# Xharlie/BtcDet

Measured on AMD Instinct MI355X. Metric: scenes/s fwd+bwd KITTI-Car bs=2/GPU (BtcDet hot path), higher is better.
Workload: dtype f32

## Files before the change

btcdet_amd/csrc/bn.hip:

```cpp
#include "btc_common.h"
#include "bn_fuse.h"
#include "../../include/btcdet_hip_infer.h"

#include <type_traits>

namespace {

constexpr int BN_T = 256;

struct BnShape {
  int N, C, cpow, rpi;
};

__device__ __forceinline__ void st_partial(double* p, double v) { btc_st_agent(p, v); }

template <bool BF, int W>
__device__ __forceinline__ void bn_ld(const float* base, long long i, float (&e)[W]) {
  if constexpr (W == 4) {
    const float4 v = btc_ld4<BF>(base, i);
    e[0] = v.x; e[1] = v.y; e[2] = v.z; e[3] = v.w;
  } else {
    e[0] = btc_ld1<BF>(base, i);
  }
}
// ... 14 lines not shown
#pragma unroll
      for (int q = 0; q < Q; ++q) s[q][tid * W + j] = acc[q][j];
    __syncthreads();
    if (rr == 0 && cw < S.C) {
      for (int l = 1; l < S.rpi; ++l)
#pragma unroll
        for (int j = 0; j < W; ++j)
#pragma unroll
          for (int q = 0; q < Q; ++q) acc[q][j] += s[q][(tid + l * S.cpow) * W + j];
      emit(cw, acc);
    }
    __syncthreads();
  }
}

template <int W, int Q, int D, class Rows, class Done>
__device__ __forceinline__ bool bn_reduce(const BnShape& S, const BnShape& SW, double* __restrict__ partial, int32_t* __restrict__ counter,
                                          Rows rows, Done done) {
  __shared__ double s[Q][BN_T * W];
  const int G = (int)gridDim.x;
  auto at = [&](int g, int q, int c) { return &partial[((size_t)g * Q + q) * S.C + c]; };
  bn_pass<W>(SW, s,
             [&](int cw, int rr, double (&acc)[Q][W]) { rows(cw, (long long)blockIdx.x * SW.rpi + rr, (long long)G * SW.rpi, acc); },
             [&](int cw, double (&acc)[Q][W]) {
#pragma unroll
               for (int j = 0; j < W; ++j)
#pragma unroll
                 for (int q = 0; q < Q; ++q) st_partial(at(blockIdx.x, q, cw * W + j), acc[q][j]);
             });
  if (!btc_last_arriver(counter, G)) return false;
  bn_pass<1>(S, s,
             [&](int c, int rr, double (&acc)[Q][1]) {
               int g = rr;
               for (; g + (D - 1) * S.rpi < G; g += D * S.rpi) {
                 double v[Q][D];
#pragma unroll
                 for (int u = 0; u < D; ++u)
#pragma unroll
                   for (int q = 0; q < Q; ++q) v[q][u] = btc_ld_agent(at(g + u * S.rpi, q, c));
#pragma unroll
                 for (int q = 0; q < Q; ++q) {
#pragma unroll
                   for (int h = 1; h < D; h *= 2)
#pragma unroll
                     for (int u = 0; u < D; u += 2 * h) v[q][u] += v[q][u + h];
                   acc[q][0] += v[q][0];
                 }
               }
               for (; g < G; g += S.rpi)
#pragma unroll
                 for (int q = 0; q < Q; ++q) acc[q][0] += btc_ld_agent(at(g, q, c));
             },
             [&](int c, double (&acc)[Q][1]) {
               double t[Q];
#pragma unroll
               for (int q = 0; q < Q; ++q) t[q] = acc[q][0];
               done(c, t);
             });
  if (threadIdx.x == 0) __hip_atomic_store(counter, 0, __ATOMIC_RELAXED, __HIP_MEMORY_SCOPE_AGENT);
  return true;
}

template <bool BF, bool VEC>
__global__ __launch_bounds__(BN_T) void bn_stats(const float* __restrict__ x, BnShape S, BnShape SW, double* __restrict__ partial,
                                                 int32_t* __restrict__ counter, float momentum, float eps, float* __restrict__ running_mean,
                                                 float* __restrict__ running_var, long long* __restrict__ num_batches,
                                                 float* __restrict__ mean_out, float* __restrict__ rstd_out) {
  constexpr int W = VEC ? 4 : 1;
  const bool last = bn_reduce<W, 2, 8>(
      S, SW, partial, counter,
      [&](int cw, long long r, long long stride, double (&acc)[2][W]) {
        const long long step = stride * S.C;
        long long i = r * S.C + cw * W;
// ... 55 lines not shown
      float g = gamma ? gamma[c + j] : 1.f, b = beta ? beta[c + j] : 0.f;
      o[j] = bn_affine(o[j], mean[c + j], rstd[c + j], g, b, relu);
    }
    btc_st4<BF>(y, i, o[0], o[1], o[2], o[3]);
  } else {
    int c = (int)(i % C);
    float g = gamma ? gamma[c] : 1.f, b = beta ? beta[c] : 0.f;
    btc_st1<BF>(y, i, bn_affine(btc_ld1<BF>(x, i), mean[c], rstd[c], g, b, relu));
  }
}

template <bool BF, bool VEC>
__global__ __launch_bounds__(BN_T) void bn_bwd_stats(const float* __restrict__ x, const float* __restrict__ y, const float* __restrict__ dy,
                                                     const float* __restrict__ mean, const float* __restrict__ rstd, BnShape S, BnShape SW, int relu,
                                                     double* __restrict__ partial, int32_t* __restrict__ counter,
                                                     float* __restrict__ dgamma, float* __restrict__ dbeta) {
  constexpr int W = VEC ? 4 : 1, U = VEC ? 2 : 4;
  bn_reduce<W, 2, 8>(
      S, SW, partial, counter,
      [&](int cw, long long r, long long stride, double (&acc)[2][W]) {
        float m[W], rs[W];
#pragma unroll
        for (int j = 0; j < W; ++j) { m[j] = mean[cw * W + j]; rs[j] = rstd[cw * W + j]; }
        const long long step = stride * S.C;
        long long i = r * S.C + cw * W;
        for (; r + (U - 1) * stride < S.N; r += U * stride, i += U * step) {
          float gv[U][W], yv[U][W], xv[U][W];
#pragma unroll
          for (int u = 0; u < U; ++u) {
            bn_ld<BF>(dy, i + u * step, gv[u]);
            bn_ld<BF>(y, i + u * step, yv[u]);
// ... 12 lines not shown
          float gv[W], yv[W], xv[W];
          bn_ld<BF>(dy, i, gv);
          bn_ld<BF>(y, i, yv);
          bn_ld<BF>(x, i, xv);
#pragma unroll
          for (int j = 0; j < W; ++j) {
            const float g = (relu && !(yv[j] > 0.f)) ? 0.f : gv[j];
            acc[0][j] += (double)g;
            acc[1][j] += (double)g * ((xv[j] - m[j]) * rs[j]);
          }
        }
      },
      [&](int c, const double (&t)[2]) {
        dbeta[c] = (float)t[0];
        dgamma[c] = (float)t[1];
      });
}

template <bool VEC, bool BF>
__global__ __launch_bounds__(BN_T) void bn_bwd_apply(const float* __restrict__ x, const float* __restrict__ y, const float* __restrict__ dy,
                                                     const float* __restrict__ mean, const float* __restrict__ rstd,
                                                     const float* __restrict__ gamma, const float* __restrict__ dgamma,
                                                     const float* __restrict__ dbeta, long long total, int C, int N, int relu, int training,
                                                     float* __restrict__ dx) {
  long long i = ((long long)blockIdx.x * blockDim.x + threadIdx.x) * (VEC ? 4 : 1);
  if (i >= total) return;
  const float invn = 1.0f / (float)N;
  constexpr int W = VEC ? 4 : 1;
  float xv[W], yv[W], gv[W];
  if (VEC) {
    float4 a = btc_ld4<BF>(x, i), b = btc_ld4<BF>(y, i), c4 = btc_ld4<BF>(dy, i);
    xv[0] = a.x; xv[W > 1 ? 1 : 0] = a.y; xv[W > 2 ? 2 : 0] = a.z; xv[W > 3 ? 3 : 0] = a.w;
    yv[0] = b.x; yv[W > 1 ? 1 : 0] = b.y; yv[W > 2 ? 2 : 0] = b.z; yv[W > 3 ? 3 : 0] = b.w;
    gv[0] = c4.x; gv[W > 1 ? 1 : 0] = c4.y; gv[W > 2 ? 2 : 0] = c4.z; gv[W > 3 ? 3 : 0] = c4.w;
  } else {
    xv[0] = btc_ld1<BF>(x, i); yv[0] = btc_ld1<BF>(y, i); gv[0] = btc_ld1<BF>(dy, i);
  }
  const int c = (int)(i % C);
  float o[W];
#pragma unroll
  for (int j = 0; j < W; ++j) {
    float g = gv[j];
    if (relu && !(yv[j] > 0.f)) g = 0.f;
    const float gm = gamma ? gamma[c + j] : 1.f, rs = rstd[c + j];
    if (training) {
      float xh = (xv[j] - mean[c + j]) * rs;
      o[j] = gm * rs * (g - dbeta[c + j] * invn - xh * dgamma[c + j] * invn);
    } else {
      o[j] = gm * rs * g;
    }
  }
  if (VEC) btc_st4<BF>(dx, i, o[0], o[W > 1 ? 1 : 0], o[W > 2 ? 2 : 0], o[W > 3 ? 3 : 0]);
  else btc_st1<BF>(dx, i, o[0]);
}

template <bool BF>
__global__ __launch_bounds__(BN_T) void col_sum(const float* __restrict__ x, BnShape S, double* __restrict__ partial,
                                                int32_t* __restrict__ counter, float* __restrict__ out) {
  bn_reduce<1, 1, 1>(
      S, S, partial, counter,
      [&](int c, long long r, long long stride, double (&acc)[1][1]) {
        for (; r + 3 * stride < S.N; r += 4 * stride) {
          float v0 = btc_ld1<BF>(x, r * S.C + c), v1 = btc_ld1<BF>(x, (r + stride) * S.C + c), v2 = btc_ld1<BF>(x, (r + 2 * stride) * S.C + c),
                v3 = btc_ld1<BF>(x, (r + 3 * stride) * S.C + c);
          acc[0][0] += ((double)v0 + (double)v1) + ((double)v2 + (double)v3);
        }
        for (; r < S.N; r += stride) acc[0][0] += (double)btc_ld1<BF>(x, r * S.C + c);
      },
// ... 39 lines not shown
};

template <class F>
int bn_by_width(int N, int C, F&& f) {
  if ((C & 3) == 0) return f(std::integral_constant<int, 4>(), bn_shape(N, C >> 2));
  return f(std::integral_constant<int, 1>(), bn_shape(N, C));
}

}

extern "C" size_t btc_bn_ws_bytes(int C) { return 256 + btc_align((size_t)512 * 2 * C * sizeof(double)); }

template <bool BF>
static int bn_fwd_impl(const float* x, int N, int C, const float* gamma, const float* beta, float* running_mean,
                               float* running_var, long long* num_batches_tracked, float momentum, float eps, int training, int relu,
                               float* y, float* save_mean, float* save_rstd, void* ws_, size_t ws_bytes, void* stream_, bool have_stats = false) {
  hipStream_t stream = (hipStream_t)stream_;
  BTC_CHECK_ARG(N >= 1 && C >= 1, "btc_bn_relu_fwd: empty input");
  BTC_CHECK_ARG(ws_bytes >= btc_bn_ws_bytes(C), "btc_bn_relu_fwd: workspace too small");
  BTC_CHECK_ARG(training || (running_mean && running_var), "btc_bn_relu_fwd: eval mode needs running statistics");
  const BnWs ws(ws_);
  const BnShape S = bn_shape(N, C);
  const long long total = (long long)N * C;
  return bn_by_width(N, C, [&](auto w, const BnShape& SW) {
    constexpr int W = decltype(w)::value;
    if (!have_stats && training) {
      const int g = W == 4 ? bn_grid_bytes(total * (BF ? 2 : 4), BTC_TUNE_BN_FWD_KB, 64) : bn_grid(N, S);
      bn_stats<BF, W == 4><<<g, BN_T, 0, stream>>>(x, S, SW, ws.partial, ws.counter, momentum, eps, running_mean, running_var,
                                                    num_batches_tracked, save_mean, save_rstd);
    } else if (!have_stats) {
      bn_eval_stats<<<btc_cdiv(C, BN_T), BN_T, 0, stream>>>(running_mean, running_var, C, eps, save_mean, save_rstd);
    }
    BTC_LAUNCH_CHECK();
    bn_apply<W == 4, BF><<<btc_cdiv(total / W, BN_T), BN_T, 0, stream>>>(x, save_mean, save_rstd, gamma, beta, total, C, relu, y);
    BTC_LAUNCH_CHECK();
    return BTC_OK;
  });
}

template <bool BF>
static int bn_bwd_impl(const float* x, const float* y, const float* dy, int N, int C, const float* gamma, const float* save_mean,
                               const float* save_rstd, int training, int relu, float* dx, float* dgamma, float* dbeta, void* ws_,
                               size_t ws_bytes, void* stream_) {
  hipStream_t stream = (hipStream_t)stream_;
  BTC_CHECK_ARG(N >= 1 && C >= 1, "btc_bn_relu_bwd: empty input");
  BTC_CHECK_ARG(ws_bytes >= btc_bn_ws_bytes(C), "btc_bn_relu_bwd: workspace too small");
  const BnWs ws(ws_);
  const BnShape S = bn_shape(N, C);
  const long long total = (long long)N * C;
  return bn_by_width(N, C, [&](auto w, const BnShape& SW) {
    constexpr int W = decltype(w)::value;
    const int g = W == 4 ? bn_grid_bytes(total * (BF ? 6 : 12), BTC_TUNE_BN_BWD_KB, 128) : bn_grid_bwd(N, S);
    bn_bwd_stats<BF, W == 4><<<g, BN_T, 0, stream>>>(x, y, dy, save_mean, save_rstd, S, SW, relu, ws.partial, ws.counter, dgamma, dbeta);
    BTC_LAUNCH_CHECK();
    bn_bwd_apply<W == 4, BF><<<btc_cdiv(total / W, BN_T), BN_T, 0, stream>>>(x, y, dy, save_mean, save_rstd, gamma, dgamma, dbeta, total, C, N,
                                                                             relu, training, dx);
    BTC_LAUNCH_CHECK();
    return BTC_OK;
  });
}

template <bool BF>
static int col_sum_impl(const float* x, int N, int C, float* out, void* ws_, size_t ws_bytes, void* stream_) {
  hipStream_t stream = (hipStream_t)stream_;
  BTC_CHECK_ARG(N >= 1 && C >= 1, "btc_col_sum: empty input");
  BTC_CHECK_ARG(ws_bytes >= btc_bn_ws_bytes(C), "btc_col_sum: workspace too small");
  const BnWs ws(ws_);
  const BnShape S = bn_shape(N, C);
  col_sum<BF><<<bn_grid_bwd(N, S), BN_T, 0, stream>>>(x, S, ws.partial, ws.counter, out);
// ... 48 lines not shown

extern "C" int btc_conv_bn_relu_fwd_src(int operands, const void* src, long long src_rows, const void* W, const float* bias, const int32_t* nbr,
                                        const int32_t* order, int n_rows, int K, int Cin, int Cout, void* x, const float* gamma, const float* beta,
                                        float* running_mean, float* running_var, long long* num_batches_tracked, float momentum, float eps, int relu,
                                        void* y, float* save_mean, float* save_rstd, void* ws, size_t ws_bytes, void* fuse_ws, void* stream) {
  BTC_CHECK_ARG(n_rows >= 1, "btc_conv_bn_relu_fwd: empty input");
  BTC_CHECK_ARG(operands >= BTC_OPERANDS_F32 && operands <= BTC_OPERANDS_F32_SPLIT, "btc_conv_bn_relu_fwd: operands=%d", operands);
  const bool bf = operands == BTC_OPERANDS_BF16_ACT || operands == BTC_OPERANDS_BF16;
  const bool fused = fuse_ws && Cout <= BN_FUSE_CMAX && btc_tune_get(BTC_TUNE_BN_FUSE) != 1;
  BnFuse bn = btc_bn_fuse_none();
  if (fused) {
    bn.counter = (int32_t*)fuse_ws;
    bn.slots = (double*)((char*)fuse_ws + 256);
    bn.mean_out = save_mean; bn.rstd_out = save_rstd;
    bn.running_mean = running_mean; bn.running_var = running_var; bn.num_batches = num_batches_tracked;
    bn.momentum = momentum; bn.eps = eps; bn.N = n_rows; bn.C = Cout; bn.nslots = btc_bn_fuse_nslots(n_rows);
  }
  const int rc = btc_apply("btc_conv_bn_relu_fwd_src", BTC_PASS_FWD, operands, src, src_rows, W, bias, nbr, order, n_rows, K, Cin, Cout, x,
                           (hipStream_t)stream, fused ? &bn : nullptr);
  if (rc) return rc;
  if (bf)
    return bn_fwd_impl<true>((const float*)x, n_rows, Cout, gamma, beta, running_mean, running_var, num_batches_tracked, momentum, eps, 1, relu,
                             (float*)y, save_mean, save_rstd, ws, ws_bytes, stream, fused);
  return bn_fwd_impl<false>((const float*)x, n_rows, Cout, gamma, beta, running_mean, running_var, num_batches_tracked, momentum, eps, 1, relu,
                            (float*)y, save_mean, save_rstd, ws, ws_bytes, stream, fused);
}

extern "C" int btc_conv_bn_eval_fwd(int operands, const void* src, long long src_rows, const void* W, const float* bias, const int32_t* nbr,
                                    const int32_t* order, int n_rows, int K, int Cin, int Cout, const float* gamma, const float* beta,
                                    const float* running_mean, const float* running_var, float eps, int relu, void* y, void* stream) {
  BTC_CHECK_ARG(n_rows >= 1, "btc_conv_bn_eval_fwd: empty input");
  BTC_CHECK_ARG(operands >= BTC_OPERANDS_F32 && operands <= BTC_OPERANDS_F32_SPLIT, "btc_conv_bn_eval_fwd: operands=%d", operands);
  BTC_CHECK_ARG(running_mean && running_var, "btc_conv_bn_eval_fwd: eval mode needs running statistics");
  BTC_CHECK_ARG(src && W && nbr && y, "btc_conv_bn_eval_fwd: null operand");
  BnFuse bn = btc_bn_fuse_none();
  bn.ev_mean = running_mean; bn.ev_var = running_var; bn.ev_gamma = gamma; bn.ev_beta = beta; bn.ev_relu = relu ? 1 : 0;
  bn.eps = eps; bn.N = n_rows; bn.C = Cout;
  return btc_apply("btc_conv_bn_eval_fwd", BTC_PASS_FWD, operands, src, src_rows, W, bias, nbr, order, n_rows, K, Cin, Cout, y, (hipStream_t)stream, &bn);
}
```

btcdet_amd/csrc/bn_fuse.h:

```cpp
#pragma once
#include "btc_common.h"

constexpr int BN_FUSE_SLOTS_MAX = 512;
constexpr int BN_FUSE_CMAX = 1024;

struct BnFuse {
  double* slots;
  int32_t* counter;
  float* mean_out;
  float* rstd_out;
  float* running_mean;
  float* running_var;
  long long* num_batches;
  float momentum, eps;
  int N, C;
  int nslots;
  const float* ev_mean;
  const float* ev_var;
  const float* ev_gamma;
  const float* ev_beta;
  int ev_relu;
};

static inline size_t btc_bn_fuse_bytes() { return 256 + (size_t)BN_FUSE_SLOTS_MAX * 2 * BN_FUSE_CMAX * sizeof(double); }

static inline int btc_bn_fuse_nslots(long long n_rows) {
  int s = 32;
  while (s < BN_FUSE_SLOTS_MAX && (long long)s * 1024 < n_rows) s <<= 1;
  return s;
}

static inline BnFuse btc_bn_fuse_none() {
  BnFuse b;
  b.slots = nullptr; b.counter = nullptr; b.mean_out = b.rstd_out = b.running_mean = b.running_var = nullptr; b.num_batches = nullptr;
  b.momentum = b.eps = 0.f; b.N = b.C = 0; b.nslots = 32;
  b.ev_mean = b.ev_var = b.ev_gamma = b.ev_beta = nullptr; b.ev_relu = 0;
  return b;
}

__device__ __forceinline__ float bn_rstd_eval(float running_var, float eps) { return 1.0f / sqrtf(__fadd_rn(running_var, eps)); }

__device__ __forceinline__ float bn_affine(float v, float mean, float rstd, float g, float b, int relu) {
  const float t = __fadd_rn(__fmul_rn(__fmul_rn(__fsub_rn(v, mean), rstd), g), b);
  return relu ? fmaxf(t, 0.f) : t;
}

struct BnEvalCol { float m, rs, g, b; };
__device__ __forceinline__ BnEvalCol bn_eval_col(const BnFuse& bn, int col) {
  BnEvalCol k;
  const bool in = col < bn.C;
// ... 17 lines not shown
      s2 += x * x;
    }
    s1 += __shfl_xor(s1, 16, 64);
    s2 += __shfl_xor(s2, 16, 64);
    s1 += __shfl_xor(s1, 32, 64);
    s2 += __shfl_xor(s2, 32, 64);
    const int col = col0 + nt * 16 + lane;
    if (lane < 16 && col < bn.C) {
      double* p = bn.slots + ((size_t)slot * 2) * BN_FUSE_CMAX + col;
      unsafeAtomicAdd(p, s1);
      unsafeAtomicAdd(p + BN_FUSE_CMAX, s2);
    }
  }
}

__device__ __forceinline__ void bn_fuse_finish(const BnFuse& bn, int* s_flag, double* s_part = nullptr) {
  const int tid = threadIdx.x;
  asm volatile("s_waitcnt vmcnt(0)" ::: "memory");
  __syncthreads();
  if (tid == 0) {
    const int total = (int)(gridDim.x * gridDim.y * gridDim.z);
    *s_flag = (btc_ticket_take(bn.counter) == total - 1);
  }
  __syncthreads();
  if (!*s_flag) return;
  if (tid == 0) btc_ticket_acquire();
  __syncthreads();
  auto publish = [&](int c, double a, double b) {
    const double mean = a / bn.N;
    double var = b / bn.N - mean * mean;
    if (var < 0.0) var = 0.0;
    bn.mean_out[c] = (float)mean;
    bn.rstd_out[c] = (float)(1.0 / sqrt(var + (double)bn.eps));
    if (bn.running_mean) {
      const double unb = bn.N > 1 ? var * ((double)bn.N / (double)(bn.N - 1)) : var;
      bn.running_mean[c] = (float)((1.0 - bn.momentum) * bn.running_mean[c] + bn.momentum * mean);
      bn.running_var[c] = (float)((1.0 - bn.momentum) * bn.running_var[c] + bn.momentum * unb);
    }
  };
  const int T = (int)blockDim.x;
  if (s_part && bn.C <= T) {
    const int G = T / bn.C;
    const int c = tid % bn.C, g = tid / bn.C;
    double a = 0.0, b = 0.0;
    if (g < G)
      for (int s = g; s < bn.nslots; s += G) {
        double* p = bn.slots + ((size_t)s * 2) * BN_FUSE_CMAX + c;
        a += btc_ld_agent(p);
        b += btc_ld_agent(p + BN_FUSE_CMAX);
        p[0] = 0.0;
        p[BN_FUSE_CMAX] = 0.0;
      }
    s_part[2 * tid] = a;
    s_part[2 * tid + 1] = b;
// ... 29 lines not shown
```

btcdet_amd/csrc/btc_common.h:

```cpp
#pragma once
#include <hip/hip_runtime.h>
#include <stdint.h>
#include <stdio.h>

#include "../../include/btcdet_hip.h"

#define BTC_EMPTY_KEY (-1)
#define BTC_EMPTY_IDX 0x7F7F7F7F

void btc_set_error(const char* fmt, ...);

#define BTC_CHECK_ARG(cond, ...)            \
  do {                                      \
    if (!(cond)) {                          \
      btc_set_error(__VA_ARGS__);           \
      return BTC_EINVAL;                    \
    }                                       \
  } while (0)

#define BTC_HIP(call)                                                             \
  do {                                                                            \
    hipError_t e_ = (call);                                                       \
    if (e_ != hipSuccess) {                                                       \
      btc_set_error("%s failed: %s (%s:%d)", #call, hipGetErrorString(e_), __FILE__, __LINE__); \
// ... 25 lines not shown
__device__ __forceinline__ void btc_ticket_acquire() { __builtin_amdgcn_fence(__ATOMIC_ACQUIRE, "agent"); }
__device__ __forceinline__ bool btc_last_arriver(int32_t* counter, int total) {
  __shared__ int s_last;
  asm volatile("s_waitcnt vmcnt(0)" ::: "memory");
  __syncthreads();
  if (threadIdx.x == 0) s_last = (btc_ticket_take(counter) == total - 1);
  __syncthreads();
  if (!s_last) return false;
  if (threadIdx.x == 0) btc_ticket_acquire();
  __syncthreads();
  return true;
}
#endif

#define BTC_TUNE_KEYS 24
int btc_tune_get(int key);

bool btc_apply_glds_supported(int K, int Cred, int Cres);
bool btc_apply_glds_has_shape(int shape, bool bf = false);
size_t btc_apply_glds_lds_bytes(int shape, int kc, int K, bool bf, int stages = 3);
int btc_apply_glds_stages(int shape, int kc, int K, bool bf, int asked);
int btc_launch_apply_glds(bool trans_w, int shape, int kc, int xcd, bool bf, const void* feat, const float* W, const float* bias,
                          const int32_t* nbr, const int32_t* order , int n_rows, int K, int Cred, int Cres, void* out,
                          hipStream_t stream, const struct BnFuse* bn = nullptr );

int btc_apply(const char* who, int pass, int operands, const void* src, long long src_rows, const void* W, const float* bias, const int32_t* nbr,
              const int32_t* order, int n_rows, int K, int Cin, int Cout, void* dst, hipStream_t stream, const struct BnFuse* bn);

int btc_apply_bf16w(const void* src, const void* Wq, const float* bias, const int32_t* nbr, const int32_t* order, int n_rows, int K, int Cred,
                    int Cres, void* dst, hipStream_t stream, int mirror = 0, const struct BnFuse* bn = nullptr);
// ... 112 lines not shown
```

btcdet_amd/csrc/conv_apply_bf16.hip:

```cpp
#include "conv_tile.h"

namespace {

__device__ unsigned short g_zero_row_b[128];

constexpr int B_STAGES = 3;

template <int WR, int WC, int NTW, int KC, bool PAIR = false>
__global__ __launch_bounds__(64 * WR * WC) void conv_apply_b(const unsigned short* __restrict__ feat, const unsigned short* __restrict__ Wq,
                                                             const float* __restrict__ bias, const int32_t* __restrict__ nbr,
                                                             const int32_t* __restrict__ order, int n_rows, int K, int Cred, int Cres,
                                                             unsigned short* __restrict__ out, int flags, const BnFuse bn) {
  extern __shared__ __attribute__((aligned(16))) char smem[];
  constexpr int NW = WR * WC, THREADS = 64 * NW;
  constexpr int TM = 16 * WR, TN = 16 * NTW * WC;
  constexpr int UPR = KC / 8;
  constexpr int RPB = (128 / (KC * 2)) < 1 ? 1 : (128 / (KC * 2));
  constexpr int A_UNITS = TM * UPR, B_UNITS = TN * UPR;
  constexpr int NAI_TOTAL = (A_UNITS + 63) / 64, NAI = (NAI_TOTAL + NW - 1) / NW;
  constexpr int NBI_TOTAL = (B_UNITS + 63) / 64, NBI = (NBI_TOTAL + NW - 1) / NW;
  constexpr int NPI = NAI + NBI;
  constexpr int A_BYTES = (TM * KC * 2 + 1023) / 1024 * 1024;
  constexpr int B_BYTES = (TN * KC * 2 + 1023) / 1024 * 1024;
  constexpr int STAGE = A_BYTES + B_BYTES;
// ... 85 lines not shown
        for (int nt = 0; nt < NTW; ++nt)
          acc[nt] = __builtin_amdgcn_mfma_f32_16x16x32_bf16(a[s], b[s][nt], acc[nt], 0, 0, 0);
      }
    }
    st = (st == B_STAGES - 1) ? 0 : st + 1;
  }

  float vals[NTW][4];
  bool valid[4];
  int rows[4];
#pragma unroll
  for (int r = 0; r < 4; ++r) rows[r] = s_row[wr * 16 + kq * 4 + r];
  apply_tile_epilogue<NTW>(acc, rows, n0 + wc * NTW * 16, bias, Cres, out, bn, bn.ev_mean != nullptr, vals, valid);
  if (bn.slots) {
    bn_fuse_wave<NTW>(bn, vals, valid, n0 + wc * NTW * 16, (int)((bx * WR + wr) & (bn.nslots - 1)));
    bn_fuse_finish(bn, (int*)smem, (double*)(smem + 16));
  }
}

size_t lds_bytes_b(int tm, int tn, int kc, int K) {
  const size_t a = ((size_t)tm * kc * 2 + 1023) / 1024 * 1024, b = ((size_t)tn * kc * 2 + 1023) / 1024 * 1024;
  return (size_t)B_STAGES * (a + b) + apply_tail_bytes(tm, K);
}

template <int WR, int WC, int NTW, int KC, bool PAIR = false>
int launch_b(const unsigned short* feat, const unsigned short* Wq, const float* bias, const int32_t* nbr, const int32_t* order, int n_rows, int K, int Cred,
             int Cres, unsigned short* out, int flags, hipStream_t stream, const BnFuse& bn) {
  constexpr int TM = 16 * WR, TN = 16 * NTW * WC;
  return apply_launch<conv_apply_b<WR, WC, NTW, KC, PAIR>>("conv_apply_b", dim3(btc_cdiv(n_rows, TM), Cres / TN), 64 * WR * WC, lds_bytes_b(TM, TN, KC, K),
                                                          stream, feat, Wq, bias, nbr, order, n_rows, K, Cred, Cres, out, flags, bn);
}
// ... 89 lines not shown
```

btcdet_amd/csrc/conv_apply_glds.hip:

```cpp
#include "conv_tile.h"

namespace {

__device__ float g_zero_row[64];

constexpr int G_STAGES_DEFAULT = 3;
constexpr int G_STAGES_MAX = 8;

__device__ __forceinline__ void transpose4(const f32x4 v, float& y0, float& y1, float& y2, float& y3) {
  unsigned x0 = __float_as_uint(v[0]), x1 = __float_as_uint(v[1]), x2 = __float_as_uint(v[2]), x3 = __float_as_uint(v[3]);
  auto a = __builtin_amdgcn_permlane32_swap(x0, x2, false, false);
  x0 = a[0]; x2 = a[1];
  auto b = __builtin_amdgcn_permlane32_swap(x1, x3, false, false);
  x1 = b[0]; x3 = b[1];
  auto c = __builtin_amdgcn_permlane16_swap(x0, x1, false, false);
  x0 = c[0]; x1 = c[1];
  auto d = __builtin_amdgcn_permlane16_swap(x2, x3, false, false);
  x2 = d[0]; x3 = d[1];
  y0 = __uint_as_float(x0); y1 = __uint_as_float(x1); y2 = __uint_as_float(x2); y3 = __uint_as_float(x3);
}

template <int WR, int WC, int NTW, bool TRANS_W, int KC, bool BF>
__global__ __launch_bounds__(64 * WR * WC) void conv_apply_g(const void* __restrict__ feat_, const float* __restrict__ W,
                                                             const float* __restrict__ bias, const int32_t* __restrict__ nbr,
// ... 162 lines not shown
      }
    }
    st = (st == S - 1) ? 0 : st + 1;
  }

  float vals[NTW][4];
  bool valid[4];
  int rows[4];
#pragma unroll
  for (int r = 0; r < 4; ++r) rows[r] = s_row[wr * 16 + kq * 4 + r];
  const bool ev = !TRANS_W && bn.ev_mean != nullptr;
  typedef typename std::conditional<BF, unsigned short, float>::type OUT;
  apply_tile_epilogue<NTW>(acc, rows, n0 + wc * NTW * 16, bias, Cres, (OUT*)out_, bn, ev, vals, valid);
  if (bn.slots) {
    bn_fuse_wave<NTW>(bn, vals, valid, n0 + wc * NTW * 16, (int)((bx * WR + wr) & (bn.nslots - 1)));
    bn_fuse_finish(bn, (int*)smem, (double*)(smem + 16));
  }
}

template <int WR, int WC, int NTW, bool TRANS_W, int KC, bool BF>
int launch_g(const void* feat, const float* W, const float* bias, const int32_t* nbr, const int32_t* order, int n_rows, int K, int Cred,
             int Cres, void* out, int xcd, hipStream_t stream, const BnFuse& bn) {
  constexpr int TM = 16 * WR, TN = 16 * NTW * WC;
  const int stages = btc_apply_glds_stages(WR * 100 + WC * 10 + NTW, KC, K, BF, (xcd >> APPLY_STAGES_SHIFT) & 15);
  xcd = (xcd & (APPLY_XCD | APPLY_MIRROR)) | (stages << APPLY_STAGES_SHIFT);
  const size_t lds = btc_apply_glds_lds_bytes(WR * 100 + WC * 10 + NTW, KC, K, BF, stages);
  return apply_launch<conv_apply_g<WR, WC, NTW, TRANS_W, KC, BF>>("conv_apply_g", dim3(btc_cdiv(n_rows, TM), Cres / TN), 64 * WR * WC, lds, stream, feat, W,
                                                                  bias, nbr, order, n_rows, K, Cred, Cres, out, xcd,
                                                                  btc_tune_get(BTC_TUNE_APPLY_DEBUG), bn);
}

// ... 88 lines not shown
```

btcdet_amd/csrc/conv_apply_split.hip:

```cpp
#include "conv_tile.h"

namespace {

#define BTC_RSRC_RECORDS 0xFFFFFF00u
#define BTC_RSRC_ABSENT 0xFFFFFFF0u
__device__ __forceinline__ void blds16s(__amdgpu_buffer_rsrc_t rsrc, unsigned voffset, void* l) {
  __builtin_amdgcn_raw_ptr_buffer_load_lds(rsrc, (__attribute__((address_space(3))) void*)l, 16, voffset, 0, 0, 0);
}

template <int WR, int WC, int NTW, int KC, int S_STAGES, int LW, bool PAIR = false>
__global__ __launch_bounds__(64 * (WR * WC + LW)) void conv_apply_s(const float* __restrict__ feat, const unsigned short* __restrict__ Ws,
                                                             const float* __restrict__ bias, const int32_t* __restrict__ nbr,
                                                             const int32_t* __restrict__ order, int n_rows, int K, int Cred, int Cres,
                                                             float* __restrict__ out, int flags, const BnFuse bn) {
  extern __shared__ __attribute__((aligned(16))) char smem[];
  constexpr int NW = WR * WC, THREADS = 64 * (NW + LW);
  constexpr int NLD = LW ? LW : NW;
  constexpr int TM = 16 * WR, TN = 16 * NTW * WC;
  constexpr int UPA = KC / 4, UPB = KC / 8;
  constexpr int A_UNITS = TM * UPA, B_UNITS = 3 * TN * UPB;
  static_assert(A_UNITS % 64 == 0 && B_UNITS % 64 == 0, "whole DMA instructions");
  constexpr int NAI_TOTAL = A_UNITS / 64, NAI = (NAI_TOTAL + NLD - 1) / NLD;
  constexpr int NBI_TOTAL = B_UNITS / 64, NBI = (NBI_TOTAL + NLD - 1) / NLD;
  static_assert(LW == 0 || (NAI_TOTAL % LW == 0 && NBI_TOTAL % LW == 0), "the loader waves share the pieces evenly");
// ... 196 lines not shown
      if (ev) ec = bn_eval_col(bn, col);
#pragma unroll
      for (int r = 0; r < 4; ++r) {
        const int row = s_row[wr * 16 + kg * 4 + r];
        valid[r] = row >= 0;
        const float sum = acc[nt][r] + (accm[nt][r] + accs[nt][r]);
        float v = bias ? (sum + bv0) : sum;
        if (ev) v = bn_affine(v, ec.m, ec.rs, ec.g, ec.b, bn.ev_relu);
        if (row >= 0) out[(size_t)row * Cres + col] = v;
        vals[nt][r] = v;
      }
    }
  }
  if (bn.slots) {
    if (computes) bn_fuse_wave<NTW>(bn, vals, valid, n0 + wc * NTW * 16, (int)((bx * WR + wr) & (bn.nslots - 1)));
    bn_fuse_finish(bn, (int*)smem, (double*)(smem + 16));
  }
}

size_t lds_bytes_s(int tm, int tn, int kc, int K, int stages) {
  return (size_t)stages * ((size_t)tm * kc * 4 + (size_t)3 * tn * kc * 2) + apply_tail_bytes(tm, K);
}

template <int WR, int WC, int NTW, int KC, int S_STAGES, int LW = 0, bool PAIR = false>
int launch_s(const float* feat, const unsigned short* Ws, const float* bias, const int32_t* nbr, const int32_t* order, int n_rows, int K, int Cred,
             int Cres, float* out, int flags, hipStream_t stream, const BnFuse& bn, int zsplit) {
  constexpr int TM = 16 * WR, TN = 16 * NTW * WC;
  return apply_launch<conv_apply_s<WR, WC, NTW, KC, S_STAGES, LW, PAIR>>("conv_apply_s", dim3(btc_cdiv(n_rows, TM), Cres / TN, zsplit), 64 * (WR * WC + LW),
                                                                        lds_bytes_s(TM, TN, KC, K, S_STAGES), stream, feat, Ws, bias, nbr, order, n_rows, K,
                                                                        Cred, Cres, out, flags, bn);
}
// ... 36 lines not shown
  }
  if (bn.slots) {
    const int slot = (int)((blockIdx.x * 4 + wave) & (bn.nslots - 1));
#pragma unroll
    for (int e = 0; e < 4; ++e) {
      s1[e] += __shfl_xor(s1[e], 16, 64);
      s2[e] += __shfl_xor(s2[e], 16, 64);
      s1[e] += __shfl_xor(s1[e], 32, 64);
      s2[e] += __shfl_xor(s2[e], 32, 64);
      if (lane < 16 && col + e < bn.C) {
        double* p = bn.slots + ((size_t)slot * 2) * BN_FUSE_CMAX + col + e;
        unsafeAtomicAdd(p, s1[e]);
        unsafeAtomicAdd(p + BN_FUSE_CMAX, s2[e]);
      }
    }
    bn_fuse_finish(bn, &s_flag);
  }
}

constexpr int SPLIT_MULTI_MAX = 32;
struct SplitTable {
  const float* W[SPLIT_MULTI_MAX];
  unsigned short* w_s[SPLIT_MULTI_MAX];
  unsigned short* wt_s[SPLIT_MULTI_MAX];
  int K[SPLIT_MULTI_MAX], Cin[SPLIT_MULTI_MAX], Cout[SPLIT_MULTI_MAX], first_block[SPLIT_MULTI_MAX + 1];
  int n;
};

__global__ __launch_bounds__(256) void weights_split3_multi(const SplitTable t) {
  int s = 0;
  while (s + 1 < t.n && (int)blockIdx.x >= t.first_block[s + 1]) ++s;
// ... 176 lines not shown
```

btcdet_amd/csrc/sparse_conv.hip:

```cpp
#include "conv_tile.h"

namespace {

constexpr int KC = 32;
constexpr int LDA = KC + 2;

template <int NT, bool TRANS_W, bool VEC, int KB, int THREADS>
__global__ __launch_bounds__(THREADS) void conv_apply(const float* __restrict__ feat, const float* __restrict__ W,
                                                  const float* __restrict__ bias, const int32_t* __restrict__ nbr,
                                                  int n_rows, int K, int Cred, int Cres, float* __restrict__ out, int mirror, const BnFuse bn) {
  extern __shared__ __attribute__((aligned(16))) char smem[];
  constexpr int TM = THREADS / 4;
  constexpr int LDB = ldb_of(NT);
  constexpr int NB = NT * 512 / THREADS;
  float* As = (float*)smem;
  float* Bs = As + KB * TM * LDA;
  int32_t* s_nbr = (int32_t*)(Bs + KB * KC * LDB);
  int32_t* s_kact = s_nbr + TM * K;
  int32_t* s_nact = s_kact + K;

  const int tid = threadIdx.x, lane = tid & 63, wave = tid >> 6;
  const int row0 = blockIdx.x * TM;
  const int n0 = blockIdx.y * (NT * 16);

// ... 126 lines not shown
#pragma unroll
        for (int nt = 0; nt < NT; ++nt) acc[nt] = __builtin_amdgcn_mfma_f32_16x16x4f32(a, bp[nt * 16], acc[nt], 0, 0, 0);
      }
    }
  }

  float vals[NT][4];
  bool valid[4];
  int rows[4];
#pragma unroll
  for (int r = 0; r < 4; ++r) rows[r] = row0 + wave * 16 + kq * 4 + r < n_rows ? row0 + wave * 16 + kq * 4 + r : -1;
  const bool ev = !TRANS_W && bn.ev_mean != nullptr;
  apply_tile_epilogue<NT, true>(acc, rows, n0, bias, Cres, out, bn, ev, vals, valid);
  if (bn.slots) {
    bn_fuse_wave<NT>(bn, vals, valid, n0, (int)((blockIdx.x * (THREADS / 64) + wave) & (bn.nslots - 1)));
    bn_fuse_finish(bn, (int*)smem, (double*)(smem + 16));
  }
}

constexpr int WS_WAVES = 16;
constexpr int WS_KB = 8;
constexpr int WS_Q = 2;

__host__ __device__ inline size_t ws_lds_bytes(int K, int Cred, int nt) {
  int crp = (Cred + 3) & ~3;
  return (size_t)K * crp * (nt * 16) * sizeof(float) + (size_t)WS_WAVES * 16 * K * sizeof(int32_t);
}

template <int NT, bool TRANS_W, bool EV = false>
__global__ __launch_bounds__(WS_WAVES * 64) void conv_apply_ws(const float* __restrict__ feat, const float* __restrict__ W,
                                                              const float* __restrict__ bias, const int32_t* __restrict__ nbr,
// ... 99 lines not shown
      const int col = nt * 16 + lrow;
      const float bv0 = (bias && col < Cres) ? bias[col] : 0.f;
      BnEvalCol ec = {0.f, 0.f, 1.f, 0.f};
      if (ev) ec = bn_eval_col(bn, col);
#pragma unroll
      for (int r = 0; r < 4; ++r) {
        const int row = row0 + kq * 4 + r;
        vals[nt][r] = bias ? (acc[nt][r] + bv0) : acc[nt][r];
        if (ev) vals[nt][r] = bn_affine(vals[nt][r], ec.m, ec.rs, ec.g, ec.b, bn.ev_relu);
        if (col < Cres && row < n_rows) out[(size_t)row * Cres + col] = vals[nt][r];
      }
    }
    if (bn.slots) bn_fuse_wave<NT>(bn, vals, valid, 0, (int)(tile & (bn.nslots - 1)));
    __builtin_amdgcn_wave_barrier();
  }
  if (bn.slots) bn_fuse_finish(bn, (int*)smem, (double*)(smem + 16));
}


__global__ __launch_bounds__(256) void maxpool_fwd_k(const float* __restrict__ feat, const int32_t* __restrict__ nbr,
                                                     int n_out, int K, int C, float* __restrict__ out) {
  long long t = (long long)blockIdx.x * blockDim.x + threadIdx.x;
  if (t >= (long long)n_out * C) return;
  int i = (int)(t / C), c = (int)(t % C);
  float m = 0.f;
  for (int k = 0; k < K; ++k) {
    int j = nbr[(size_t)i * K + k];
    if (j >= 0) m = fmaxf(m, feat[(size_t)j * C + c]);
  }
  out[t] = m;
}
// ... 243 lines not shown
```

Before: 590.7.

## Hand off BN stat reduction to apply kernels instead of last-arriver ticket

Replaces the last-arriver ticket finish, both in the fused conv+BN forward path and in the BN backward stats kernel, with a handoff. The stats kernels now only write per-block partials. A grid-limited apply kernel then reduces the slots or partials in its prologue and applies the normalization, which removes the serialized tail work done by one block. When ticket mode is off, the slot count is capped so the prologue reads stay small. The cost is that every apply block re-reads the partials, plus a new strided apply loop with a capped grid.

After: 599.2, median of 6. 1.01x the previous value.

```diff
diff --git a/btcdet_amd/csrc/bn.hip b/btcdet_amd/csrc/bn.hip
--- a/btcdet_amd/csrc/bn.hip
+++ b/btcdet_amd/csrc/bn.hip
@@ -52,9 +52,43 @@
   }
 }
 
+template <int Q, int D, bool AGENT, int SW_, class Done>
+__device__ __forceinline__ void bn_gather(const BnShape& S, int G, const double* __restrict__ partial, double (&s)[Q][SW_], Done done) {
+  auto at = [&](int g, int q, int c) { return &partial[((size_t)g * Q + q) * S.C + c]; };
+  auto ld = [&](const double* p) { return AGENT ? btc_ld_agent(p) : *p; };
+  bn_pass<1>(S, s,
+             [&](int c, int rr, double (&acc)[Q][1]) {
+               int g = rr;
+               for (; g + (D - 1) * S.rpi < G; g += D * S.rpi) {
+                 double v[Q][D];
+#pragma unroll
+                 for (int u = 0; u < D; ++u)
+#pragma unroll
+                   for (int q = 0; q < Q; ++q) v[q][u] = ld(at(g + u * S.rpi, q, c));
+#pragma unroll
+                 for (int q = 0; q < Q; ++q) {
+#pragma unroll
+                   for (int h = 1; h < D; h *= 2)
+#pragma unroll
+                     for (int u = 0; u < D; u += 2 * h) v[q][u] += v[q][u + h];
+                   acc[q][0] += v[q][0];
+                 }
+               }
+               for (; g < G; g += S.rpi)
+#pragma unroll
+                 for (int q = 0; q < Q; ++q) acc[q][0] += ld(at(g, q, c));
+             },
+             [&](int c, double (&acc)[Q][1]) {
+               double t[Q];
+#pragma unroll
+               for (int q = 0; q < Q; ++q) t[q] = acc[q][0];
+               done(c, t);
+             });
+}
+
 template <int W, int Q, int D, class Rows, class Done>
 __device__ __forceinline__ bool bn_reduce(const BnShape& S, const BnShape& SW, double* __restrict__ partial, int32_t* __restrict__ counter,
-                                          Rows rows, Done done) {
+                                          Rows rows, Done done, bool handoff = false) {
   __shared__ double s[Q][BN_T * W];
   const int G = (int)gridDim.x;
   auto at = [&](int g, int q, int c) { return &partial[((size_t)g * Q + q) * S.C + c]; };
@@ -66,35 +100,9 @@
 #pragma unroll
                  for (int q = 0; q < Q; ++q) st_partial(at(blockIdx.x, q, cw * W + j), acc[q][j]);
              });
+  if (handoff) return false;
   if (!btc_last_arriver(counter, G)) return false;
-  bn_pass<1>(S, s,
-             [&](int c, int rr, double (&acc)[Q][1]) {
-               int g = rr;
-               for (; g + (D - 1) * S.rpi < G; g += D * S.rpi) {
-                 double v[Q][D];
-#pragma unroll
-                 for (int u = 0; u < D; ++u)
-#pragma unroll
-                   for (int q = 0; q < Q; ++q) v[q][u] = btc_ld_agent(at(g + u * S.rpi, q, c));
-#pragma unroll
-                 for (int q = 0; q < Q; ++q) {
-#pragma unroll
-                   for (int h = 1; h < D; h *= 2)
-#pragma unroll
-                     for (int u = 0; u < D; u += 2 * h) v[q][u] += v[q][u + h];
-                   acc[q][0] += v[q][0];
-                 }
-               }
-               for (; g < G; g += S.rpi)
-#pragma unroll
-                 for (int q = 0; q < Q; ++q) acc[q][0] += btc_ld_agent(at(g, q, c));
-             },
-             [&](int c, double (&acc)[Q][1]) {
-               double t[Q];
-#pragma unroll
-               for (int q = 0; q < Q; ++q) t[q] = acc[q][0];
-               done(c, t);
-             });
+  bn_gather<Q, D, true>(S, G, partial, s, done);
   if (threadIdx.x == 0) __hip_atomic_store(counter, 0, __ATOMIC_RELAXED, __HIP_MEMORY_SCOPE_AGENT);
   return true;
 }
@@ -180,7 +188,7 @@
 __global__ __launch_bounds__(BN_T) void bn_bwd_stats(const float* __restrict__ x, const float* __restrict__ y, const float* __restrict__ dy,
                                                      const float* __restrict__ mean, const float* __restrict__ rstd, BnShape S, BnShape SW, int relu,
                                                      double* __restrict__ partial, int32_t* __restrict__ counter,
-                                                     float* __restrict__ dgamma, float* __restrict__ dbeta) {
+                                                     float* __restrict__ dgamma, float* __restrict__ dbeta, int handoff) {
   constexpr int W = VEC ? 4 : 1, U = VEC ? 2 : 4;
   bn_reduce<W, 2, 8>(
       S, SW, partial, counter,
@@ -223,7 +231,19 @@
       [&](int c, const double (&t)[2]) {
         dbeta[c] = (float)t[0];
         dgamma[c] = (float)t[1];
-      });
+      },
+      handoff != 0);
+}
+
+__device__ __forceinline__ float bn_bwd_dx(float x, float y, float dy, float mean, float rs, float gm, float dgamma, float dbeta, float invn,
+                                           int relu, int training) {
+  float g = dy;
+  if (relu && !(y > 0.f)) g = 0.f;
+  if (training) {
+    float xh = (x - mean) * rs;
+    return gm * rs * (g - dbeta * invn - xh * dgamma * invn);
+  }
+  return gm * rs * g;
 }
 
 template <bool VEC, bool BF>
@@ -249,18 +269,196 @@
   float o[W];
 #pragma unroll
   for (int j = 0; j < W; ++j) {
-    float g = gv[j];
-    if (relu && !(yv[j] > 0.f)) g = 0.f;
-    const float gm = gamma ? gamma[c + j] : 1.f, rs = rstd[c + j];
-    if (training) {
-      float xh = (xv[j] - mean[c + j]) * rs;
-      o[j] = gm * rs * (g - dbeta[c + j] * invn - xh * dgamma[c + j] * invn);
-    } else {
-      o[j] = gm * rs * g;
-    }
+    const float gm = gamma ? gamma[c + j] : 1.f;
+    o[j] = training ? bn_bwd_dx(xv[j], yv[j], gv[j], mean[c + j], rstd[c + j], gm, dgamma[c + j], dbeta[c + j], invn, relu, 1)
+                    : bn_bwd_dx(xv[j], yv[j], gv[j], 0.f, rstd[c + j], gm, 0.f, 0.f, invn, relu, 0);
   }
   if (VEC) btc_st4<BF>(dx, i, o[0], o[W > 1 ? 1 : 0], o[W > 2 ? 2 : 0], o[W > 3 ? 3 : 0]);
   else btc_st1<BF>(dx, i, o[0]);
+}
+
+constexpr int BN_HANDOFF_WGS = 512;
+constexpr int BN_FWD_U = 4;
+constexpr int BN_HANDOFF_CMAX = 1024;
+constexpr int BN_HANDOFF_BYTES = 64 * 1024;
+static_assert(BN_HANDOFF_CMAX == BN_FUSE_CMAX, "bn_apply_finish's tables hold every fused channel count");
+
+template <int W, int U, class Load, class Prologue, class Store>
+__device__ __forceinline__ void bn_strided(long long total, int C, Load load, Prologue prologue, Store store) {
+  const long long nv = total / W, stride = (long long)gridDim.x * BN_T;
+  long long v = (long long)blockIdx.x * BN_T + threadIdx.x;
+  int c = (int)((v * W) % C);
+  const int cs = (int)((stride * W) % C);
+  int cu[U];
+  auto loads = [&]() {
+#pragma unroll
+    for (int u = 0; u < U; ++u) {
+      cu[u] = c;
+      if (v + u * stride < nv) load((v + u * stride) * W, u);
+      c += cs;
+      if (c >= C) c -= C;
+    }
+    __builtin_amdgcn_sched_barrier(0);
+  };
+  auto stores = [&]() {
+#pragma unroll
+    for (int u = 0; u < U; ++u)
+      if (v + u * stride < nv) store((v + u * stride) * W, cu[u], u);
+  };
+  loads();
+  prologue();
+  stores();
+  for (v += U * stride; v < nv; v += U * stride) {
+    loads();
+    stores();
+  }
+}
+
+int bn_handoff_grid(long long vectors, int U) {
+  const long long g = btc_cdiv(vectors, (long long)BN_T * U);
+  return (int)(g > BN_HANDOFF_WGS ? BN_HANDOFF_WGS : (g < 1 ? 1 : g));
+}
+
+template <bool VEC, bool BF>
+__global__ __launch_bounds__(BN_T) void bn_apply_finish(const float* __restrict__ x, const float* __restrict__ gamma, const float* __restrict__ beta,
+                                                        long long total, int relu, float* __restrict__ y, const BnFuse bn) {
+  constexpr int W = VEC ? 4 : 1;
+  __shared__ double s_sum[2][BN_HANDOFF_CMAX];
+  __shared__ double s_part[2][BN_T];
+  __shared__ float s_k[4][BN_HANDOFF_CMAX];
+  __shared__ int s_last;
+  const int tid = threadIdx.x, C = bn.C;
+  auto slot = [&](int s, int c) { return bn.slots + ((size_t)s * 2) * BN_FUSE_CMAX + c; };
+  auto prologue = [&]() {
+    for (int c = tid; c < C; c += BN_T) {
+      s_k[2][c] = gamma ? gamma[c] : 1.f;
+      s_k[3][c] = beta ? beta[c] : 0.f;
+    }
+    if (C <= BN_T) {
+      const int G = BN_T / C;
+      const int c = tid % C, g = tid / C;
+      double a = 0.0, b = 0.0;
+      constexpr int SB = 16;
+      if (g < G) {
+        for (int s0 = g; s0 < bn.nslots; s0 += SB * G) {
+          double va[SB], vb[SB];
+#pragma unroll
+          for (int u = 0; u < SB; ++u) {
+            const int s = s0 + u * G;
+            const bool in = s < bn.nslots;
+            va[u] = in ? *slot(s, c) : 0.0;
+            vb[u] = in ? *(slot(s, c) + BN_FUSE_CMAX) : 0.0;
+          }
+#pragma unroll
+          for (int u = 0; u < SB; ++u) {
+            a += va[u];
+            b += vb[u];
+          }
+        }
+      }
+      s_part[0][tid] = a;
+      s_part[1][tid] = b;
+      __syncthreads();
+      if (tid < C) {
+        a = b = 0.0;
+        for (int q = 0; q < G; ++q) {
+          a += s_part[0][q * C + tid];
+          b += s_part[1][q * C + tid];
+        }
+        s_sum[0][tid] = a;
+        s_sum[1][tid] = b;
+      }
+    } else {
+      for (int c = tid; c < C; c += BN_T) {
+        double a = 0.0, b = 0.0;
+#pragma unroll 8
+        for (int s = 0; s < bn.nslots; ++s) {
+          a += *slot(s, c);
+          b += *(slot(s, c) + BN_FUSE_CMAX);
+        }
+        s_sum[0][c] = a;
+        s_sum[1][c] = b;
+      }
+    }
+    for (int c = tid; c < C; c += BN_T) {
+      const BnMoments m = bn_fuse_moments(s_sum[0][c], s_sum[1][c], bn.N, bn.eps);
+      s_k[0][c] = (float)m.mean;
+      s_k[1][c] = m.rstd;
+    }
+    __syncthreads();
+    if (tid == 0) s_last = (btc_ticket_take(bn.counter) == (int)gridDim.x - 1);
+  };
+
+  float e[BN_FWD_U][W];
+  bn_strided<W, BN_FWD_U>(
+      total, C, [&](long long i, int u) { bn_ld<BF>(x, i, e[u]); }, prologue,
+      [&](long long i, int c, int u) {
+        float o[W];
+#pragma unroll
+        for (int j = 0; j < W; ++j) o[j] = bn_affine(e[u][j], s_k[0][c + j], s_k[1][c + j], s_k[2][c + j], s_k[3][c + j], relu);
+        if constexpr (VEC) btc_st4<BF>(y, i, o[0], o[W > 1 ? 1 : 0], o[W > 2 ? 2 : 0], o[W > 3 ? 3 : 0]);
+        else btc_st1<BF>(y, i, o[0]);
+      });
+
+  __syncthreads();
+  if (!s_last) return;
+  for (int c = tid; c < C; c += BN_T) bn_fuse_publish(bn, c, bn_fuse_moments(s_sum[0][c], s_sum[1][c], bn.N, bn.eps));
+  for (int i = tid; i < bn.nslots * C; i += BN_T) {
+    double* p = slot(i / C, i % C);
+    p[0] = 0.0;
+    p[BN_FUSE_CMAX] = 0.0;
+  }
+  if (tid == 0) {
+    if (bn.num_batches) *bn.num_batches += 1;
+    __hip_atomic_store(bn.counter, 0, __ATOMIC_RELAXED, __HIP_MEMORY_SCOPE_AGENT);
+  }
+}
+
+template <bool VEC, bool BF>
+__global__ __launch_bounds__(BN_T) void bn_bwd_apply_gather(const float* __restrict__ x, const float* __restrict__ y, const float* __restrict__ dy,
+                                                            const float* __restrict__ mean, const float* __restrict__ rstd,
+                                                            const float* __restrict__ gamma, const double* __restrict__ partial, int G,
+                                                            BnShape S, long long total, int relu, int training,
+                                                            float* __restrict__ dgamma, float* __restrict__ dbeta, float* __restrict__ dx) {
+  constexpr int W = VEC ? 4 : 1, U = VEC ? 2 : 4;
+  __shared__ double s[2][BN_T];
+  __shared__ float s_k[5][BN_HANDOFF_CMAX];
+  const int tid = threadIdx.x, C = S.C;
+  auto prologue = [&]() {
+    for (int c = tid; c < C; c += BN_T) {
+      s_k[0][c] = mean[c];
+      s_k[1][c] = rstd[c];
+      s_k[2][c] = gamma ? gamma[c] : 1.f;
+    }
+    bn_gather<2, 8, false>(S, G, partial, s, [&](int c, const double (&t)[2]) {
+      s_k[4][c] = (float)t[0];
+      s_k[3][c] = (float)t[1];
+      if (blockIdx.x == 0) {
+        dbeta[c] = (float)t[0];
+        dgamma[c] = (float)t[1];
+      }
+    });
+    __syncthreads();
+  };
+  const float invn = 1.0f / (float)S.N;
+  float xv[U][W], yv[U][W], gv[U][W];
+  bn_strided<W, U>(
+      total, C,
+      [&](long long i, int u) {
+        bn_ld<BF>(x, i, xv[u]);
+        bn_ld<BF>(y, i, yv[u]);
+        bn_ld<BF>(dy, i, gv[u]);
+      },
+      prologue,
+      [&](long long i, int c, int u) {
+        float o[W];
+#pragma unroll
+        for (int j = 0; j < W; ++j)
+          o[j] = bn_bwd_dx(xv[u][j], yv[u][j], gv[u][j], s_k[0][c + j], s_k[1][c + j], s_k[2][c + j], s_k[3][c + j], s_k[4][c + j], invn, relu,
+                           training);
+        if constexpr (VEC) btc_st4<BF>(dx, i, o[0], o[W > 1 ? 1 : 0], o[W > 2 ? 2 : 0], o[W > 3 ? 3 : 0]);
+        else btc_st1<BF>(dx, i, o[0]);
+      });
 }
 
 template <bool BF>
@@ -330,7 +528,8 @@
 template <bool BF>
 static int bn_fwd_impl(const float* x, int N, int C, const float* gamma, const float* beta, float* running_mean,
                                float* running_var, long long* num_batches_tracked, float momentum, float eps, int training, int relu,
-                               float* y, float* save_mean, float* save_rstd, void* ws_, size_t ws_bytes, void* stream_, bool have_stats = false) {
+                               float* y, float* save_mean, float* save_rstd, void* ws_, size_t ws_bytes, void* stream_, const BnFuse* fused = nullptr) {
+  const bool have_stats = fused != nullptr;
   hipStream_t stream = (hipStream_t)stream_;
   BTC_CHECK_ARG(N >= 1 && C >= 1, "btc_bn_relu_fwd: empty input");
   BTC_CHECK_ARG(ws_bytes >= btc_bn_ws_bytes(C), "btc_bn_relu_fwd: workspace too small");
@@ -348,6 +547,11 @@
       bn_eval_stats<<<btc_cdiv(C, BN_T), BN_T, 0, stream>>>(running_mean, running_var, C, eps, save_mean, save_rstd);
     }
     BTC_LAUNCH_CHECK();
+    if (fused && !fused->ticket) {
+      bn_apply_finish<W == 4, BF><<<bn_handoff_grid(total / W, BN_FWD_U), BN_T, 0, stream>>>(x, gamma, beta, total, relu, y, *fused);
+      BTC_LAUNCH_CHECK();
+      return BTC_OK;
+    }
     bn_apply<W == 4, BF><<<btc_cdiv(total / W, BN_T), BN_T, 0, stream>>>(x, save_mean, save_rstd, gamma, beta, total, C, relu, y);
     BTC_LAUNCH_CHECK();
     return BTC_OK;
@@ -367,8 +571,17 @@
   return bn_by_width(N, C, [&](auto w, const BnShape& SW) {
     constexpr int W = decltype(w)::value;
     const int g = W == 4 ? bn_grid_bytes(total * (BF ? 6 : 12), BTC_TUNE_BN_BWD_KB, 128) : bn_grid_bwd(N, S);
-    bn_bwd_stats<BF, W == 4><<<g, BN_T, 0, stream>>>(x, y, dy, save_mean, save_rstd, S, SW, relu, ws.partial, ws.counter, dgamma, dbeta);
+    const bool handoff = C <= BN_HANDOFF_CMAX && (long long)g * C * 2 * (long long)sizeof(double) <= BN_HANDOFF_BYTES &&
+                         btc_tune_get(BTC_TUNE_BN_TICKET) != 1;
+    bn_bwd_stats<BF, W == 4><<<g, BN_T, 0, stream>>>(x, y, dy, save_mean, save_rstd, S, SW, relu, ws.partial, ws.counter, dgamma, dbeta,
+                                                     handoff ? 1 : 0);
     BTC_LAUNCH_CHECK();
+    if (handoff) {
+      bn_bwd_apply_gather<W == 4, BF><<<bn_handoff_grid(total / W, W == 4 ? 2 : 4), BN_T, 0, stream>>>(x, y, dy, save_mean, save_rstd, gamma, ws.partial, g, S, total, relu, training,
+                                                                  dgamma, dbeta, dx);
+      BTC_LAUNCH_CHECK();
+      return BTC_OK;
+    }
     bn_bwd_apply<W == 4, BF><<<btc_cdiv(total / W, BN_T), BN_T, 0, stream>>>(x, y, dy, save_mean, save_rstd, gamma, dgamma, dbeta, total, C, N,
                                                                              relu, training, dx);
     BTC_LAUNCH_CHECK();
@@ -447,16 +660,18 @@
     bn.slots = (double*)((char*)fuse_ws + 256);
     bn.mean_out = save_mean; bn.rstd_out = save_rstd;
     bn.running_mean = running_mean; bn.running_var = running_var; bn.num_batches = num_batches_tracked;
-    bn.momentum = momentum; bn.eps = eps; bn.N = n_rows; bn.C = Cout; bn.nslots = btc_bn_fuse_nslots(n_rows);
+    bn.momentum = momentum; bn.eps = eps; bn.N = n_rows; bn.C = Cout;
+    bn.ticket = btc_tune_get(BTC_TUNE_BN_TICKET) == 1;
+    bn.nslots = btc_bn_fuse_nslots(n_rows, Cout, bn.ticket);
   }
   const int rc = btc_apply("btc_conv_bn_relu_fwd_src", BTC_PASS_FWD, operands, src, src_rows, W, bias, nbr, order, n_rows, K, Cin, Cout, x,
                            (hipStream_t)stream, fused ? &bn : nullptr);
   if (rc) return rc;
   if (bf)
     return bn_fwd_impl<true>((const float*)x, n_rows, Cout, gamma, beta, running_mean, running_var, num_batches_tracked, momentum, eps, 1, relu,
-                             (float*)y, save_mean, save_rstd, ws, ws_bytes, stream, fused);
+                             (float*)y, save_mean, save_rstd, ws, ws_bytes, stream, fused ? &bn : nullptr);
   return bn_fwd_impl<false>((const float*)x, n_rows, Cout, gamma, beta, running_mean, running_var, num_batches_tracked, momentum, eps, 1, relu,
-                            (float*)y, save_mean, save_rstd, ws, ws_bytes, stream, fused);
+                            (float*)y, save_mean, save_rstd, ws, ws_bytes, stream, fused ? &bn : nullptr);
 }
 
 extern "C" int btc_conv_bn_eval_fwd(int operands, const void* src, long long src_rows, const void* W, const float* bias, const int32_t* nbr,
diff --git a/btcdet_amd/csrc/bn_fuse.h b/btcdet_amd/csrc/bn_fuse.h
--- a/btcdet_amd/csrc/bn_fuse.h
+++ b/btcdet_amd/csrc/bn_fuse.h
@@ -15,6 +15,7 @@
   float momentum, eps;
   int N, C;
   int nslots;
+  int ticket;
   const float* ev_mean;
   const float* ev_var;
   const float* ev_gamma;
@@ -24,16 +25,20 @@
 
 static inline size_t btc_bn_fuse_bytes() { return 256 + (size_t)BN_FUSE_SLOTS_MAX * 2 * BN_FUSE_CMAX * sizeof(double); }
 
-static inline int btc_bn_fuse_nslots(long long n_rows) {
+constexpr int BN_FUSE_PROLOGUE_BYTES = 64 * 1024;
+static inline int btc_bn_fuse_nslots(long long n_rows, int C = 0, int ticket = 1) {
+  int cap = BN_FUSE_SLOTS_MAX;
+  if (!ticket)
+    while (cap > 32 && (long long)cap * C * 2 * (int)sizeof(double) > BN_FUSE_PROLOGUE_BYTES) cap >>= 1;
   int s = 32;
-  while (s < BN_FUSE_SLOTS_MAX && (long long)s * 1024 < n_rows) s <<= 1;
+  while (s < cap && (long long)s * 1024 < n_rows) s <<= 1;
   return s;
 }
 
 static inline BnFuse btc_bn_fuse_none() {
   BnFuse b;
   b.slots = nullptr; b.counter = nullptr; b.mean_out = b.rstd_out = b.running_mean = b.running_var = nullptr; b.num_batches = nullptr;
-  b.momentum = b.eps = 0.f; b.N = b.C = 0; b.nslots = 32;
+  b.momentum = b.eps = 0.f; b.N = b.C = 0; b.nslots = 32; b.ticket = 0;
   b.ev_mean = b.ev_var = b.ev_gamma = b.ev_beta = nullptr; b.ev_relu = 0;
   return b;
 }
@@ -81,6 +86,25 @@
   }
 }
 
+struct BnMoments { double mean, var; float rstd; };
+__device__ __forceinline__ BnMoments bn_fuse_moments(double a, double b, int N, float eps) {
+  BnMoments m;
+  m.mean = a / N;
+  m.var = b / N - m.mean * m.mean;
+  if (m.var < 0.0) m.var = 0.0;
+  m.rstd = (float)(1.0 / sqrt(m.var + (double)eps));
+  return m;
+}
+__device__ __forceinline__ void bn_fuse_publish(const BnFuse& bn, int c, const BnMoments& m) {
+  bn.mean_out[c] = (float)m.mean;
+  bn.rstd_out[c] = m.rstd;
+  if (bn.running_mean) {
+    const double unb = bn.N > 1 ? m.var * ((double)bn.N / (double)(bn.N - 1)) : m.var;
+    bn.running_mean[c] = (float)((1.0 - bn.momentum) * bn.running_mean[c] + bn.momentum * m.mean);
+    bn.running_var[c] = (float)((1.0 - bn.momentum) * bn.running_var[c] + bn.momentum * unb);
+  }
+}
+
 __device__ __forceinline__ void bn_fuse_finish(const BnFuse& bn, int* s_flag, double* s_part = nullptr) {
   const int tid = threadIdx.x;
   asm volatile("s_waitcnt vmcnt(0)" ::: "memory");
@@ -93,18 +117,7 @@
   if (!*s_flag) return;
   if (tid == 0) btc_ticket_acquire();
   __syncthreads();
-  auto publish = [&](int c, double a, double b) {
-    const double mean = a / bn.N;
-    double var = b / bn.N - mean * mean;
-    if (var < 0.0) var = 0.0;
-    bn.mean_out[c] = (float)mean;
-    bn.rstd_out[c] = (float)(1.0 / sqrt(var + (double)bn.eps));
-    if (bn.running_mean) {
-      const double unb = bn.N > 1 ? var * ((double)bn.N / (double)(bn.N - 1)) : var;
-      bn.running_mean[c] = (float)((1.0 - bn.momentum) * bn.running_mean[c] + bn.momentum * mean);
-      bn.running_var[c] = (float)((1.0 - bn.momentum) * bn.running_var[c] + bn.momentum * unb);
-    }
-  };
+  auto publish = [&](int c, double a, double b) { bn_fuse_publish(bn, c, bn_fuse_moments(a, b, bn.N, bn.eps)); };
   const int T = (int)blockDim.x;
   if (s_part && bn.C <= T) {
     const int G = T / bn.C;
diff --git a/btcdet_amd/csrc/btc_common.h b/btcdet_amd/csrc/btc_common.h
--- a/btcdet_amd/csrc/btc_common.h
+++ b/btcdet_amd/csrc/btc_common.h
@@ -63,6 +63,7 @@
 #endif
 
 #define BTC_TUNE_KEYS 24
+#define BTC_TUNE_BN_TICKET 16
 int btc_tune_get(int key);
 
 bool btc_apply_glds_supported(int K, int Cred, int Cres);
diff --git a/btcdet_amd/csrc/conv_apply_bf16.hip b/btcdet_amd/csrc/conv_apply_bf16.hip
--- a/btcdet_amd/csrc/conv_apply_bf16.hip
+++ b/btcdet_amd/csrc/conv_apply_bf16.hip
@@ -123,7 +123,7 @@
   apply_tile_epilogue<NTW>(acc, rows, n0 + wc * NTW * 16, bias, Cres, out, bn, bn.ev_mean != nullptr, vals, valid);
   if (bn.slots) {
     bn_fuse_wave<NTW>(bn, vals, valid, n0 + wc * NTW * 16, (int)((bx * WR + wr) & (bn.nslots - 1)));
-    bn_fuse_finish(bn, (int*)smem, (double*)(smem + 16));
+    if (bn.ticket) bn_fuse_finish(bn, (int*)smem, (double*)(smem + 16));
   }
 }
 
diff --git a/btcdet_amd/csrc/conv_apply_glds.hip b/btcdet_amd/csrc/conv_apply_glds.hip
--- a/btcdet_amd/csrc/conv_apply_glds.hip
+++ b/btcdet_amd/csrc/conv_apply_glds.hip
@@ -200,7 +200,7 @@
   apply_tile_epilogue<NTW>(acc, rows, n0 + wc * NTW * 16, bias, Cres, (OUT*)out_, bn, ev, vals, valid);
   if (bn.slots) {
     bn_fuse_wave<NTW>(bn, vals, valid, n0 + wc * NTW * 16, (int)((bx * WR + wr) & (bn.nslots - 1)));
-    bn_fuse_finish(bn, (int*)smem, (double*)(smem + 16));
+    if (bn.ticket) bn_fuse_finish(bn, (int*)smem, (double*)(smem + 16));
   }
 }
 
diff --git a/btcdet_amd/csrc/conv_apply_split.hip b/btcdet_amd/csrc/conv_apply_split.hip
--- a/btcdet_amd/csrc/conv_apply_split.hip
+++ b/btcdet_amd/csrc/conv_apply_split.hip
@@ -234,7 +234,7 @@
   }
   if (bn.slots) {
     if (computes) bn_fuse_wave<NTW>(bn, vals, valid, n0 + wc * NTW * 16, (int)((bx * WR + wr) & (bn.nslots - 1)));
-    bn_fuse_finish(bn, (int*)smem, (double*)(smem + 16));
+    if (bn.ticket) bn_fuse_finish(bn, (int*)smem, (double*)(smem + 16));
   }
 }
 
@@ -301,7 +301,7 @@
         unsafeAtomicAdd(p + BN_FUSE_CMAX, s2[e]);
       }
     }
-    bn_fuse_finish(bn, &s_flag);
+    if (bn.ticket) bn_fuse_finish(bn, &s_flag);
   }
 }
 
diff --git a/btcdet_amd/csrc/sparse_conv.hip b/btcdet_amd/csrc/sparse_conv.hip
--- a/btcdet_amd/csrc/sparse_conv.hip
+++ b/btcdet_amd/csrc/sparse_conv.hip
@@ -164,7 +164,7 @@
   apply_tile_epilogue<NT, true>(acc, rows, n0, bias, Cres, out, bn, ev, vals, valid);
   if (bn.slots) {
     bn_fuse_wave<NT>(bn, vals, valid, n0, (int)((blockIdx.x * (THREADS / 64) + wave) & (bn.nslots - 1)));
-    bn_fuse_finish(bn, (int*)smem, (double*)(smem + 16));
+    if (bn.ticket) bn_fuse_finish(bn, (int*)smem, (double*)(smem + 16));
   }
 }
 
@@ -294,7 +294,7 @@
     if (bn.slots) bn_fuse_wave<NT>(bn, vals, valid, 0, (int)(tile & (bn.nslots - 1)));
     __builtin_amdgcn_wave_barrier();
   }
-  if (bn.slots) bn_fuse_finish(bn, (int*)smem, (double*)(smem + 16));
+  if (bn.slots && bn.ticket) bn_fuse_finish(bn, (int*)smem, (double*)(smem + 16));
 }
 
 
```
